# titoeb/RecModel

Hardware: AMD Instinct MI355X
Metric: ALS user+item row-updates/sec (higher is better)
Workload: dtype f32; 1 GPU; cfg3: WMF k=128+bias, 10000000x1000000 CSR, 99990947 nnz, alpha-log confidence, gamma=0.1, zipf_a=0.0; n_items=1000000, nnz=99990947, k=128, bias=True

## Files before the change

### include/wmf_hip.h

```cpp
#ifndef WMF_HIP_H
#define WMF_HIP_H

#include <stdint.h>

#ifdef __cplusplus
extern "C" {
#endif

#define WMF_OK            0
#define WMF_EINVAL       -1
#define WMF_EHIP         -2
#define WMF_ENOMEM       -3
#define WMF_ENUMERIC     -4

#define WMF_MAX_F        260

typedef struct wmf_plan wmf_plan;

const char* wmf_last_error(void);
int  wmf_version(void);
int  wmf_ld_for(int f);

int wmf_recompute_factors_host(const float* Y_host, int64_t m, int f, int bias,
                               const int64_t* indptr, const int32_t* indices, const float* values,
// ... 1 lines not shown

int64_t wmf_gram_workspace_bytes(int f);

int wmf_gram(const float* Y, int64_t m, int f, int ld, int bias,
             double* G_sum, void* workspace, void* stream);

int wmf_factorize(const double* G_sum, int f, int ld, double lambda,
                  float* W_white, float* W_unwhite, int32_t* info,
                  void* workspace, void* stream);

int wmf_rolled_layout_supported(int f, int ld);

int wmf_row_transform(const float* in, int64_t m, int f, int ld, const float* W,
                      int set_col0_one, float* out, float* col0_out, void* stream);
int wmf_whitened_row_floats(int f, int ld, int bias);

int  wmf_plan_create(const int64_t* indptr_host, int64_t n, int f, int bias, wmf_plan** out);
void wmf_plan_destroy(wmf_plan* p);
int  wmf_plan_stats(const wmf_plan* p, int64_t* out14);
int  wmf_plan_iter_stats(wmf_plan* p, int64_t* out4);

int wmf_solve_rows(const wmf_plan* plan, const float* V, const float* bias_fixed,
                   const int64_t* indptr, const int32_t* indices, const float* values,
                   int64_t n, int f, int ld, float* g, int32_t* fail_count, void* stream);
#define WMF_SOLVE_ROLLED 1
int wmf_solve_rows_ex(const wmf_plan* plan, const float* V, const float* bias_fixed,
                   const int64_t* indptr, const int32_t* indices, const float* values,
                   int64_t n, int f, int ld, float* g, int32_t* fail_count, int flags, void* stream);

int64_t wmf_eval_workspace_bytes(void);
// ... 133 lines not shown
```

### recmodel_amd/_lib.py

```python
import ctypes
import os

import torch

_HERE = os.path.dirname(os.path.abspath(__file__))
LIB_PATH = os.environ.get("WMF_HIP_LIB", os.path.join(_HERE, "libwmf_hip.so"))

WMF_OK, WMF_EINVAL, WMF_EHIP, WMF_ENOMEM, WMF_ENUMERIC = 0, -1, -2, -3, -4

c_int, c_i64, c_dbl, c_vp = ctypes.c_int, ctypes.c_int64, ctypes.c_double, ctypes.c_void_p

SIGNATURES = {
    "wmf_last_error": (ctypes.c_char_p, []),
    "wmf_version": (c_int, []),
    "wmf_ld_for": (c_int, [c_int]),
    "wmf_recompute_factors_host": (c_int, [c_vp, c_i64, c_int, c_int, c_vp, c_vp, c_vp, c_i64, c_dbl, c_vp]),
    "wmf_gram_workspace_bytes": (c_i64, [c_int]),
    "wmf_gram": (c_int, [c_vp, c_i64, c_int, c_int, c_int, c_vp, c_vp, c_vp]),
    "wmf_factorize": (c_int, [c_vp, c_int, c_int, c_dbl, c_vp, c_vp, c_vp, c_vp, c_vp]),
    "wmf_row_transform": (c_int, [c_vp, c_i64, c_int, c_int, c_vp, c_int, c_vp, c_vp, c_vp]),
    "wmf_whitened_row_floats": (c_int, [c_int, c_int, c_int]),
    "wmf_plan_create": (c_int, [c_vp, c_i64, c_int, c_int, ctypes.POINTER(c_vp)]),
    "wmf_plan_destroy": (None, [c_vp]),
    "wmf_plan_stats": (c_int, [c_vp, c_vp]),
    "wmf_plan_iter_stats": (c_int, [c_vp, c_vp]),
    "wmf_solve_rows": (c_int, [c_vp, c_vp, c_vp, c_vp, c_vp, c_vp, c_i64, c_int, c_int, c_vp, c_vp, c_vp]),
    "wmf_solve_rows_ex": (c_int, [c_vp, c_vp, c_vp, c_vp, c_vp, c_vp, c_i64, c_int, c_int, c_vp, c_vp, c_int, c_vp]),
    "wmf_rolled_layout_supported": (c_int, [c_int, c_int]),
    "wmf_eval_workspace_bytes": (c_i64, []),
    "wmf_eval_sqerr": (c_int, [c_vp, c_vp, c_int, c_int, c_int, c_vp, c_vp, c_vp, c_i64, c_vp, c_vp, c_vp]),
    "wmf_audit_workspace_bytes": (c_i64, [c_i64]),
    "wmf_half_step_audit": (c_int, [c_vp, c_vp, c_int, c_int, c_int, c_vp, c_vp, c_vp, c_i64, c_vp, c_vp, c_vp, c_vp, c_i64, c_vp]),
    "wmf_half_step_audit_f64": (c_int, [c_vp, c_vp, c_int, c_int, c_vp, c_vp, c_vp, c_i64, c_vp, c_vp, c_vp, c_vp, c_i64, c_vp]),
    "wmf_predict_pairs": (c_int, [c_vp, c_vp, c_int, c_int, c_int, c_vp, c_i64, c_vp, c_i64, c_vp, c_vp]),
    "wmf_partial_row_floats": (c_i64, [c_int]),
    "wmf_accumulate_rows": (c_int, [c_vp, c_vp, c_vp, c_vp, c_vp, c_vp, c_i64, c_i64, c_int, c_int, c_vp, c_int, c_int, c_vp, c_vp]),
# ... 130 lines not shown
```

### recmodel_amd/csrc/wmf_api.hip

```cpp
#include "../../include/wmf_hip.h"
#include "wmf_internal.h"

#include <atomic>
#include <cstdarg>
#include <cstdio>
#include <cstring>
#include <mutex>
#include <set>
#include <string>
#include <vector>

static thread_local char g_err[512] = "";
int wmf_debug_flags = 0;

void wmf_set_error(const char* fmt, ...) {
    va_list ap;
    va_start(ap, fmt);
    vsnprintf(g_err, sizeof(g_err), fmt, ap);
    va_end(ap);
}

#define HIP_TRY(call)                                                                            \
    do {                                                                                         \
        hipError_t e_ = (call);                                                                  \
// ... 197 lines not shown
    return check_launch("wmf_factorize");
}

int wmf_row_transform(const float* in, int64_t m, int f, int ld, const float* W, int set_col0_one, float* out,
                      float* col0_out, void* stream) {
    int rc = check_shape(f, ld);
    if (rc) return rc;
    if (!in || !W || !out || m < 0) { wmf_set_error("wmf_row_transform: null pointer or negative m"); return WMF_EINVAL; }
    rc = wmf_launch_transform(in, m, f, ld, W, set_col0_one, out, col0_out, (hipStream_t)stream);
    if (rc) {
        if (rc == WMF_L_LAYOUT) wmf_set_error("wmf_row_transform: f=%d, ld=%d with set_col0_one writes the split layout: col0_out (float[2 m]) is required and out may not alias in", f, ld);
        else wmf_set_error("wmf_row_transform: unsupported f=%d", f);
        return WMF_EINVAL;
    }
    return check_launch("wmf_row_transform");
}

static int bin_of(int64_t d, int f) {
    if (d <= 16) return WMF_BIN_LOW16;
    if (d <= 32) return WMF_BIN_LOW32;
    return wmf_direct_supported(f) ? WMF_BIN_MFMA : WMF_BIN_GENERAL;
}

int wmf_plan_create(const int64_t* indptr, int64_t n, int f, int bias, wmf_plan** out) {
    if (!indptr || !out || n < 0 || n > 0x7fffffffLL) { wmf_set_error("wmf_plan_create: bad arguments"); return WMF_EINVAL; }
    if (f < 1 || f > WMF_MAX_F) { wmf_set_error("wmf_plan_create: f=%d unsupported", f); return WMF_EINVAL; }
    wmf_plan* p = new wmf_plan();
    memset(p, 0, sizeof(*p));
    p->n = n; p->f = f;
    std::vector<int32_t> order((size_t)n);
// ... 558 lines not shown
```

### recmodel_amd/csrc/wmf_dense.hip

```cpp
#include "wmf_common.h"
#include "wmf_internal.h"

#include <type_traits>
#include <utility>

template <int NFB, int NSPLIT, int S>
__device__ __forceinline__ void gram_body(const float* __restrict__ Y, int64_t m, int f, int ld, int bias,
                                          float* __restrict__ partial, int64_t step_lo, int64_t step_hi) {
    constexpr int NT = NFB * (NFB + 1) / 2;
    constexpr int NACC = (NT + NSPLIT - 1) / NSPLIT;
    const int lane = threadIdx.x & 63;
    const int r = lane & 15, q = lane >> 4;
    f32x4 acc[NACC];
#pragma unroll
    for (int i = 0; i < NACC; ++i) acc[i] = f32x4{0.f, 0.f, 0.f, 0.f};

    constexpr int U = 4;
    float cur[U][NFB], nxt[U][NFB];
    const int last_col = min(16 * (NFB - 1) + r, ld - 1);
    const float col_mask_last = (16 * (NFB - 1) + r < f) ? 1.f : 0.f;
    auto load_trip = [&](int64_t s0, float (&fr)[U][NFB]) {
#pragma unroll
        for (int uu = 0; uu < U; ++uu) {
            const int64_t row = min(4 * (s0 + uu) + q, m - 1);
// ... 32 lines not shown
    float* out = partial + (int64_t)blockIdx.x * NT * 256;
    int t = 0;
#pragma unroll
    for (int bi = 0; bi < NFB; ++bi) {
#pragma unroll
        for (int bj = bi; bj < NFB; ++bj, ++t) {
            if (t % NSPLIT == S) {
#pragma unroll
                for (int reg = 0; reg < 4; ++reg) out[(t * 4 + reg) * 64 + lane] = acc[t / NSPLIT][reg];
            }
        }
    }
}

typedef __bf16 gram_bf16x8 __attribute__((ext_vector_type(8)));
template <int NFB>
__device__ __forceinline__ void gram_body6(const float* __restrict__ Y, int64_t m, int f, int ld, int bias,
                                           float* __restrict__ partial, int64_t step_lo, int64_t step_hi) {
    constexpr int NT = NFB * (NFB + 1) / 2;
    constexpr int NG1 = (5 * NFB + 4) / 9;
    const int lane = threadIdx.x;
    const int r = lane & 15, q = lane >> 4;
    f32x4 acc[NT];
#pragma unroll
    for (int i = 0; i < NT; ++i) acc[i] = f32x4{0.f, 0.f, 0.f, 0.f};
    const int last_col = min(16 * (NFB - 1) + r, ld - 1);
    const float col_mask_last = (16 * (NFB - 1) + r < f) ? 1.f : 0.f;
    const bool bias_lane = bias && r == 0;
    const int64_t stride = 32 * step_hi;
    auto load_blocks = [&](int64_t c0, float (&fr)[8][NFB], int fb_lo, int fb_hi) {
#pragma unroll
        for (int j = 0; j < 8; ++j) {
            const int64_t row = min(c0 + 8 * q + j, m - 1);
            const float* yrow = Y + row * (int64_t)ld;
#pragma unroll
            for (int fb = 0; fb < NFB; ++fb)
                if (fb >= fb_lo && fb < fb_hi) fr[j][fb] = yrow[fb == NFB - 1 ? last_col : 16 * fb + r];
        }
    };
    auto split = [&](int64_t c0, const float (&fr)[8][NFB], auto masked, gram_bf16x8 (&hi)[NFB], gram_bf16x8 (&mid)[NFB],
                     gram_bf16x8 (&lo)[NFB]) {
#pragma unroll
        for (int fb = 0; fb < NFB; ++fb) {
#pragma unroll
            for (int j = 0; j < 8; ++j) {
                const float rmask = (!decltype(masked)::value || c0 + 8 * q + j < m) ? 1.f : 0.f;
                float x = fr[j][fb];
                if (decltype(masked)::value) x *= rmask;
                if (fb == NFB - 1) x *= col_mask_last;
                if (fb == 0 && bias_lane) x = rmask;
                const __bf16 h = (__bf16)x;
                const float r1 = x - (float)h;
                const __bf16 md = (__bf16)r1;
                hi[fb][j] = h; mid[fb][j] = md; lo[fb][j] = (__bf16)(r1 - (float)md);
            }
        }
    };
    auto products = [&](const gram_bf16x8 (&hi)[NFB], const gram_bf16x8 (&mid)[NFB], const gram_bf16x8 (&lo)[NFB]) {
        int t0 = 0;
#pragma unroll
        for (int bi = 0; bi < NFB; ++bi) {
#pragma unroll
            for (int bj = bi; bj < NFB; ++bj) acc[t0 + bj - bi] = __builtin_amdgcn_mfma_f32_16x16x32_bf16(lo[bi], hi[bj], acc[t0 + bj - bi], 0, 0, 0);
#pragma unroll
            for (int bj = bi; bj < NFB; ++bj) acc[t0 + bj - bi] = __builtin_amdgcn_mfma_f32_16x16x32_bf16(mid[bi], mid[bj], acc[t0 + bj - bi], 0, 0, 0);
// ... 30 lines not shown
        gram_bf16x8 hi[NFB], mid[NFB], lo[NFB];
        split(c0, cur, std::true_type{}, hi, mid, lo);
        products(hi, mid, lo);
    }
    float* out = partial + (int64_t)blockIdx.x * NT * 256;
#pragma unroll
    for (int t = 0; t < NT; ++t)
#pragma unroll
        for (int reg = 0; reg < 4; ++reg) out[(t * 4 + reg) * 64 + lane] = acc[t][reg];
}

template <int NFB>
__global__ __launch_bounds__(64) void gram6_kernel(const float* __restrict__ Y, int64_t m, int f, int ld, int bias,
                                                   float* __restrict__ partial, int64_t steps_per_wave) {
    gram_body6<NFB>(Y, m, f, ld, bias, partial, blockIdx.x, gridDim.x);
}

template <int NFB, int NSPLIT>
__global__ __launch_bounds__(NSPLIT == 1 ? 64 : 256) void gram_kernel(const float* __restrict__ Y, int64_t m, int f, int ld, int bias,
                                                  float* __restrict__ partial, int64_t steps_per_wave) {
    const int64_t nsteps = (m + 3) / 4;
    int64_t lo = (int64_t)blockIdx.x * steps_per_wave;
    int64_t hi = lo + steps_per_wave;
    if (hi > nsteps) hi = nsteps;
    if (lo > hi) lo = hi;
    if constexpr (NSPLIT == 1) {
        gram_body<NFB, 1, 0>(Y, m, f, ld, bias, partial, lo, hi);
    } else {
        switch (__builtin_amdgcn_readfirstlane(threadIdx.x >> 6)) {
            case 0: gram_body<NFB, NSPLIT, 0>(Y, m, f, ld, bias, partial, lo, hi); break;
// ... 68 lines not shown
    const int cap = wmf_gram_max_waves(f);
    if (want > cap) want = cap;
    if (want > 1024) want -= want % 1024;
    return (int)want;
}

int wmf_launch_gram(const float* Y, int64_t m, int f, int ld, int bias, double* G_sum, float* partial, double* slices,
                    hipStream_t st) {
    if (m <= 0) return hipMemsetAsync(G_sum, 0, (size_t)f * f * sizeof(double), st) == hipSuccess ? WMF_L_OK : WMF_L_NO_KERNEL;
    const int nfb = (f + 15) / 16;
    const int nwaves = wmf_gram_nwaves(m, f);
    if (const int rc = wmf_dispatch_nfb<1, 17>(nfb, [&](auto n) { return launch_gram_nfb<decltype(n)::value>(Y, m, f, ld, bias, partial, nwaves, st); })) return rc;
    WMF_LAUNCH("gram_reduce1_kernel", gram_reduce1_kernel, dim3((f * f + 255) / 256, WMF_GRAM_SLICES), dim3(256), 0, st, partial,
               nwaves, f, nfb, slices);
    WMF_LAUNCH("gram_reduce2_kernel", gram_reduce2_kernel, dim3((f * f + 255) / 256), dim3(256), 0, st, slices, f, G_sum);
    return WMF_L_OK;
}

__device__ __forceinline__ double rl_f64(double v, int lane) {
    const int lo = __builtin_amdgcn_readlane(__double2loint(v), lane);
    const int hi = __builtin_amdgcn_readlane(__double2hiint(v), lane);
    return __hiloint2double(hi, lo);
}

typedef double f64x4 __attribute__((ext_vector_type(4)));
#define WMF_MFMA16_F64(a, b, c) __builtin_amdgcn_mfma_f64_16x16x4f64((a), (b), (c), 0, 0, 0)
constexpr int FZ_LD = 66;

__device__ __forceinline__ f64x4 fz_mul_abt(const double* A, int la, const double* B, int lb, f64x4 c, int r, int q, double sign) {
#pragma unroll
// ... 516 lines not shown
    return WMF_L_OK;
}

int wmf_launch_transform(const float* in, int64_t m, int f, int ld, const float* W, int set_col0_one, float* out,
                         float* col0_out, hipStream_t st) {
    if (m <= 0) return WMF_L_OK;
    const int nfb = (f + 15) / 16;
    if (set_col0_one == 3 || set_col0_one == 4) {
        if (!wmf_rolled_layout(f, ld)) return WMF_L_NO_KERNEL;
    } else {
        set_col0_one = set_col0_one ? (wmf_split_layout(f, ld) ? 2 : 1) : 0;
    }
    if ((set_col0_one == 2 || set_col0_one == 3) && (!col0_out || in == out)) return WMF_L_LAYOUT;
    return wmf_dispatch_nfb<1, 17>(nfb, [&](auto n) { return launch_transform_nfb<decltype(n)::value>(in, m, f, ld, W, set_col0_one, out, col0_out, st); });
}
```

### recmodel_amd/csrc/wmf_internal.h

```cpp
#pragma once
#include <hip/hip_runtime.h>
#include <stdint.h>
#include <type_traits>
#include <utility>
#include "../../include/wmf_hip.h"

#define WMF_GRAM_MAX_WAVES 4096
#define WMF_EVAL_MAX_BLOCKS 2048
#define WMF_AUDIT_MAX_BLOCKS 2048
#define WMF_HEAVY_T 4096
#define WMF_SEG 2048
#define WMF_WIDE_LU_GRID 64

extern int wmf_debug_flags;
#ifdef WMF_LAB
constexpr bool WMF_LAB_BUILD = true;
#else
constexpr bool WMF_LAB_BUILD = false;
#endif
constexpr int WMF_DBG_SHIPPED = WMF_DBG_HEAVY_REG_RING | WMF_DBG_F32_GRAM | WMF_DBG_HEAVY_ONE_WAVE | WMF_DBG_F64_NO_LOW_RANK |
                                WMF_DBG_NO_ITER | WMF_DBG_F64_VALU;
constexpr int WMF_DBG_LAB = WMF_DBG_NO_ELIMINATION | WMF_DBG_NO_ACCUMULATION | WMF_DBG_NO_TILE_INVERSE | WMF_DBG_LOW32_GAUSS_JORDAN |
                            WMF_DBG_NO_BORDER | WMF_DBG_WIDE_EIGHT_WAVES | WMF_DBG_NO_ROW_PAIRS | WMF_DBG_HEAVY_F32_ACC |
                            WMF_DBG_HEAVY_REG_RING_K64 | WMF_DBG_F32_TRANSFORM | WMF_DBG_LOW_F32_TILES | WMF_DBG_WIDE_F32 |
// ... 24 lines not shown
    int64_t iter_count, iter_nnz;
    int iter_dmax;
    int32_t* iter_bounce_rows;
    int32_t* iter_info;
    unsigned long long* iter_stats;
};

int wmf_gram_max_waves(int f);
int wmf_gram_nwaves(int64_t m, int f);
int wmf_launch_gram(const float* Y, int64_t m, int f, int ld, int bias, double* G_sum, float* partial, double* slices,
                    hipStream_t st);
int wmf_launch_factorize(const double* G_sum, int f, int ld, double lambda, float* Wwhite, float* Wunwhite,
                         int32_t* info, double* gA, hipStream_t st);
int wmf_launch_transform(const float* in, int64_t m, int f, int ld, const float* W, int set_col0_one, float* out,
                         float* col0_out, hipStream_t st);

enum WmfLaunchRc { WMF_L_OK = 0, WMF_L_NO_KERNEL = -1, WMF_L_HIP = -2, WMF_L_LAYOUT = -3, WMF_L_TOO_MANY_KEYS = -4 };

struct RowArgs {
    const float* V; const float* side; const float* biasv; int bstride;
    const int64_t* indptr; const int32_t* indices; const float* vals;
    int f, ld; float* g; int32_t* fb_rows; int32_t* fb_count; int32_t* fail_count;
    int dbg; bool rolled; hipStream_t st;
};
struct RowList { const int32_t* rows; int64_t count; const int32_t* count_dev; };

template <int N>
using wmf_int = std::integral_constant<int, N>;
template <int... NS, class Fn>
static inline int wmf_dispatch_list(int n, Fn&& fn) {
// ... 152 lines not shown
```

### recmodel_amd/engine.py

```python
import ctypes
import os

import numpy as np
import torch

from . import _lib


def _ptr(t):
    return ctypes.c_void_p(t.data_ptr()) if t is not None else None


def _stream():
    return ctypes.c_void_p(torch.cuda.current_stream().cuda_stream)


class _HeldWork:

    def __init__(self, work, *buffers, landing=None):
        self.work, self.buffers, self.landing = work, buffers, landing

    def wait(self):
        self.work.wait()
        if self.landing is not None:
# ... 18 lines not shown
        return int(self.lib.wmf_gram_workspace_bytes(f))

    def eval_workspace_bytes(self):
        return int(self.lib.wmf_eval_workspace_bytes())

    def gram(self, Y, m, f, ld, bias, G, ws):
        _lib.check(self.lib.wmf_gram(_ptr(Y), m, f, ld, int(bias), _ptr(G), _ptr(ws), _stream()))

    def factorize(self, G, f, ld, lam, W_white, W_unwhite, info, ws):
        _lib.check(self.lib.wmf_factorize(_ptr(G), f, ld, float(lam), _ptr(W_white), _ptr(W_unwhite), _ptr(info), _ptr(ws),
                                          _stream()))

    def row_transform(self, inp, m, f, ld, W, set_col0_one, out, col0_out):
        _lib.check(self.lib.wmf_row_transform(_ptr(inp), m, f, ld, _ptr(W), int(set_col0_one), _ptr(out), _ptr(col0_out),
                                              _stream()))

    def plan_create(self, indptr_host, n, f, bias):
        handle = ctypes.c_void_p()
        _lib.check(self.lib.wmf_plan_create(indptr_host.ctypes.data_as(ctypes.c_void_p), n, f, int(bool(bias)), ctypes.byref(handle)))
        stats = np.zeros(14, dtype=np.int64)
        _lib.check(self.lib.wmf_plan_stats(handle, stats.ctypes.data_as(ctypes.c_void_p)))
        return handle, stats

    def plan_iter_stats(self, handle):
        out = np.zeros(4, dtype=np.int64)
        _lib.check(self.lib.wmf_plan_iter_stats(handle, out.ctypes.data_as(ctypes.c_void_p)))
        return out

    def plan_destroy(self, handle):
        self.lib.wmf_plan_destroy(handle)
# ... 234 lines not shown


def row_cost(degrees, f):
    return degrees.to(torch.float64) * float(f * f) + float(f) ** 3


def gathered_positions(ids, world, rows_per_rank, chunk_len, owner=None, local=None):
    j = ids // world if local is None else local
    r = ids % world if owner is None else owner
    s_c = (j // chunk_len) * chunk_len
    rest = rows_per_rank - s_c
    len_c = torch.clamp(rest, max=chunk_len) if torch.is_tensor(rest) else min(chunk_len, rest)
    return world * s_c + r * len_c + (j - s_c)


class AlsEngine:

    def __init__(self, n_users, n_items, dim, bias, gamma, device=None, group=None, kernels=None, chunks=None,
                 reduce_mode=None, pipe_mode=None, force_exchange=None, sparse_mode=None):
        self.K = kernels if kernels is not None else HipKernels()
        self.lib = getattr(self.K, "lib", None)
        self.device = torch.device(device if device is not None else f"cuda:{torch.cuda.current_device()}")
        self.group = group
        if group is not None or (torch.distributed.is_available() and torch.distributed.is_initialized()):
            self.world = torch.distributed.get_world_size(group)
            self.rank = torch.distributed.get_rank(group)
        else:
            self.world, self.rank = 1, 0
        if force_exchange is None:
            force_exchange = os.environ.get("WMF_FORCE_EXCHANGE") == "1"
        self.exchange = self.world > 1 or (bool(force_exchange) and torch.distributed.is_available()
                                           and torch.distributed.is_initialized())
        self.n = {"users": int(n_users), "items": int(n_items)}
        self.dim, self.bias, self.gamma = int(dim), bool(bias), float(gamma)
        self.f = self.dim + 1 if self.bias else self.dim
        self.ld = self.K.ld_for(self.f)
        self.pr = self.K.partial_row_floats(self.f) if hasattr(self.K, "partial_row_floats") else 0
        self._reduce_arg, self.pipe_mode, self._chunks_arg, self._sparse_arg = reduce_mode, pipe_mode, chunks, sparse_mode
        self.csr = {}
        self.csr_chunks = {}
        self._configure({s: Sharding(self.n[s], self.world, self.rank) for s in self.n})

    def _configure(self, shard):
        W = self.world
        self.shard = shard
        self.rpr = {s: shard[s].rpr for s in self.n}
        self.n_local = {s: shard[s].n_local for s in self.n}
        pr, chunks = self.pr, self._chunks_arg
        forced = os.environ.get("WMF_REDUCE") if self._reduce_arg is None else ("1" if self._reduce_arg else "0")
        self.reduce = {}
        for s in self.n:
            o = "items" if s == "users" else "users"
# ... 8 lines not shown
        want = {s: max(1, int(chunks)) for s in self.n}
        if auto_chunks:
            want = {s: max(1, min(want[s], (self.rpr[s] * (W if self.reduce[s] else 1)) // MIN_CHUNK_ROWS)) for s in self.n}
            for s in self.n:
                if self.reduce["items" if s == "users" else "users"]:
                    want[s] = 1
        self.chunk_len = {s: max(1, (self.rpr[s] + want[s] - 1) // want[s]) for s in self.n}
        self.chunk_bounds = {s: [(lo, min(self.chunk_len[s], self.rpr[s] - lo))
                                 for lo in range(0, max(self.rpr[s], 1), self.chunk_len[s]) if lo < self.rpr[s]]
                             for s in self.n}
        self.chunk_range = {s: [(W * lo, W * (lo + ln)) for lo, ln in self.chunk_bounds[s]] for s in self.n}
        self.sparse = {s: False for s in self.n}
        self.need = {}
        dev, f32 = self.device, torch.float32
        z = lambda *shape, dtype=f32: torch.zeros(*shape, dtype=dtype, device=dev)
        self.factors = {s: z(self.rpr[s], self.ld) for s in self.n}
        self.g = {s: z(self.rpr[s], self.ld) for s in self.n}
        self.X = {s: (z(W * self.rpr[s], self.ld) if self.exchange else self.factors[s]) for s in self.n}
        self._pending = {s: [] for s in self.n}
        self.ldv = self.K.whitened_row_floats(self.f, self.ld, self.bias)
        self.split = self.ldv != self.ld
        self.rolled = bool(self.split and self.bias and os.environ.get("WMF_ROLLED", "1") != "0"
                           and self.K.rolled_layout_supported(self.f, self.ld))
        self.white_mode = 3 if self.rolled else self.bias
        self.unwhite_mode = 4 if self.rolled else False
        self.solve_flags = 1 if self.rolled else 0
        self.V = {s: z(W * self.rpr[s], self.ldv) for s in self.n}
        self.bias_vec = {s: (z(W * self.rpr[s], 2) if self.split else z(W * self.rpr[s])) for s in self.n}
        self.G = z(self.f * self.f, dtype=torch.float64)
        self.W_white, self.W_unwhite = z(self.f, self.ld), z(self.f, self.ld)
        self.info = z(4, dtype=torch.int32)
        self.fail = z(4, dtype=torch.int32)
        self.ws = torch.empty(self.K.gram_workspace_bytes(self.f), dtype=torch.uint8, device=dev)
        self.eval_ws = torch.empty(self.K.eval_workspace_bytes(), dtype=torch.uint8, device=dev)
        self.eval_out = z(3, dtype=torch.float64)
        self.pipe = {s: False for s in self.n}
        self.csr_pipe = {}
        self.partial_pipe = {}
        self.csr_red = {}
        self.partial_all = {s: (torch.empty(W * self.rpr[s], pr, dtype=f32, device=dev) if self.reduce[s] else None) for s in self.n}
        self.partial_mine = {s: (torch.empty(self.rpr[s], pr, dtype=f32, device=dev) if self.reduce[s] else None) for s in self.n}
        self.scratch_rows = torch.zeros(max(self.rpr.values()), dtype=torch.int32, device=dev)
        self._stale = {s: False for s in self.n}
        self.csr, self.csr_chunks = {}, {}
        self.has_factors = {"users": False, "items": False}

    def positions(self, side, ids):
        sh = self.shard[side]
# ... 220 lines not shown
        indptr, idx, v = coo_to_csr(o.indices.to(torch.int64), local_rows, o.values, self.world * self.rpr[side], self.K, o.n_rows)
        deg = (indptr[1:] - indptr[:-1]).to(torch.int32).contiguous()
        w_eff = torch.empty_like(v) if self.bias and not self.split else None
        return indptr.contiguous(), deg, idx.contiguous(), v.contiguous(), w_eff

    def _shard(self, side, rows, cols, vals, plan=True):
        other = self._other(side)
        local = self.shard[side].local_of(rows)
        indptr, idx, v = coo_to_csr(local, self.positions(other, cols), vals, self.rpr[side], self.K, self.world * self.rpr[other])
        return Csr(self.K, indptr, idx, v, self.world * self.rpr[other], self.f, self.bias, plan=plan)

    def set_factors(self, side, full):
        full = torch.as_tensor(full, dtype=torch.float32)
        sh = self.shard[side]
        mine = (full[self.rank::self.world] if sh.owner is None else full[sh.my_ids(full.device)]).to(self.device)
        blk = self.factors[side]
        blk.zero_()
        blk[: mine.shape[0], : self.f] = mine
        self.has_factors[side] = True
        for c in range(len(self.chunk_bounds[side])):
            self._publish(side, c)

    def get_factors(self, side):
        ids = torch.arange(self.n[side], device=self.device)
        if self.sparse[side]:
            W = self.world
            self._wait(side)
            dense = torch.zeros(W * self.rpr[side], self.ld, dtype=torch.float32, device=self.device)
            for lo, ln in self.chunk_bounds[side]:
                torch.distributed.all_gather_into_tensor(dense[W * lo: W * (lo + ln)], self.factors[side][lo: lo + ln].contiguous(),
# ... 31 lines not shown
        return _HeldWork(work, send_h, landing=(out, out_h))

    def _ensure_gathered(self, side):
        if self._stale[side]:
            self._stale[side] = False
            for c in range(len(self.chunk_bounds[side])):
                self._publish(side, c, force=True)
        self._wait(side)

    def _wait(self, side):
        for work in self._pending[side]:
            if work is not None:
                work.wait()
        self._pending[side] = []

    def prepare(self, fixed):
        K = self.K
        blk = self.factors[fixed]
        K.gram(blk, self.n_local[fixed], self.f, self.ld, self.bias, self.G, self.ws)
        if self.exchange:
            torch.distributed.all_reduce(self.G, group=self.group)
        K.factorize(self.G, self.f, self.ld, self.gamma, self.W_white, self.W_unwhite, self.info, self.ws)
        V, bvec = self.V[fixed], self.bias_vec[fixed]
        if not self.exchange:
            K.row_transform(self.X[fixed], self.n_local[fixed], self.f, self.ld, self.W_white, self.white_mode, V,
                            bvec if self.bias else None)
            return
        if self._stale[fixed]:
            self._ensure_gathered(fixed)
        pending, self._pending[fixed] = self._pending[fixed], []
        done = len(self.chunk_bounds[fixed]) - len(pending)
        for c, (start, stop) in enumerate(self.chunk_range[fixed]):
            if c >= done and pending[c - done] is not None:
                pending[c - done].wait()
            rows = slice(start, stop)
            if stop > start:
                K.row_transform(self.X[fixed][rows], stop - start, self.f, self.ld, self.W_white, self.white_mode, V[rows],
                                bvec[rows] if self.bias else None)

    def update(self, side):
        K = self.K
        fixed = self._other(side)
        bvec = self.bias_vec[fixed] if self.bias else None
        self._wait(side)
        for c, ((lo, ln), csr) in enumerate(zip(self.chunk_bounds[side], self.csr_chunks[side])):
            g = self.g[side][lo: lo + ln]
            K.solve_rows(csr._plan, self.V[fixed], bvec, csr.indptr, csr.indices, csr.values, ln, self.f, self.ld, g, self.fail,
                         self.solve_flags)
            real = max(0, min(ln, self.n_local[side] - lo))
            K.row_transform(g, real, self.f, self.ld, self.W_unwhite, self.unwhite_mode, self.factors[side][lo: lo + ln], None)
            self._publish(side, c)
        self.has_factors[side] = True

    def half_step(self, side):
        if self.reduce[side]:
            return self._half_step_reduce(side)
        if self.pipe[side]:
            return self._half_step_pipelined(side)
        self.prepare(self._other(side))
        self.update(side)

    def _half_step_pipelined(self, side):
        K, W = self.K, self.world
        fixed = self._other(side)
        K.gram(self.factors[fixed], self.n_local[fixed], self.f, self.ld, self.bias, self.G, self.ws)
        torch.distributed.all_reduce(self.G, group=self.group)
# ... 81 lines not shown
        self.update(side)

    def _reduce_scatter(self, out, inp):
        if torch.distributed.get_backend(self.group) == "nccl":
            return torch.distributed.reduce_scatter_tensor(out, inp, group=self.group, async_op=True)
        torch.distributed.all_reduce(inp, group=self.group)
        n = out.shape[0]
        out.copy_(inp[self.rank * n: (self.rank + 1) * n])
        return None

    def half_step_unweighted(self, side):
        K = self.K
        fixed = self._other(side)
        self.prepare(fixed)
        c = self.csr[side]
        K.spmm_rows(self.V[fixed], c.indptr, c.indices, c.values, c.n_rows, self.f, self.ld, self.g[side])
        K.row_transform(self.g[side], self.n_local[side], self.f, self.ld, self.W_unwhite, self.unwhite_mode, self.factors[side], None)
        self.has_factors[side] = True
        for c in range(len(self.chunk_bounds[side])):
            self._publish(side, c)

    @property
    def iter_on(self):
        return not (_lib.load().wmf_debug_get_flags() & _lib.DEBUG_FLAGS["WMF_DBG_NO_ITER"])

    def iter_stats(self, side):
        out = np.zeros(4, dtype=np.int64)
        for c in self.csr_chunks.get(side, []):
            out += c.iter_stats()
        return out
# ... 77 lines not shown
```

Measured before the change: 422.1 million row-updates/s.

## Chain whitening transforms from solver outputs and defer factor materialization

Instead of unwhitening each solved row into factors and then re-reading those factors for the next half-step's Gram and whitening transform, the engine keeps the whitened solutions g plus the unwhitening matrix U. It computes an augmented Gram of g, composes U into the next whitening matrix on a small dense path, and applies one combined transform from g directly to V. The per-row unwhitening pass over the solved side is skipped and only materialized lazily when factors are accessed. This removes a full read/write pass over the factor matrix per half-step, at the cost of extra small compose kernels, a lazy-materialization wrapper, and possible numerical drift from the chained transforms.

After: 454.4 million row-updates/s, median of 6. 7.6% higher.

```diff
diff --git a/include/wmf_hip.h b/include/wmf_hip.h
--- a/include/wmf_hip.h
+++ b/include/wmf_hip.h
@@ -39,6 +39,15 @@
 int wmf_row_transform(const float* in, int64_t m, int f, int ld, const float* W,
                       int set_col0_one, float* out, float* col0_out, void* stream);
 int wmf_whitened_row_floats(int f, int ld, int bias);
+
+int wmf_chained_supported(int f, int ld, int bias);
+int wmf_gram_whitened(const float* g, int64_t m, int f, int ld, int bias,
+                      double* G_aug, void* workspace, void* stream);
+int wmf_compose_whitening(const double* G_aug, const float* U, int f, int ld, int bias, int rolled, double lambda,
+                          float* W_white, float* W_unwhite, float* N_ext, int32_t* info,
+                          void* workspace, void* stream);
+int wmf_row_transform_chained(const float* g, int64_t m, int f, int ld, int bias, const float* N_ext, int rolled,
+                              float* out, float* col0_out, void* stream);
 
 int  wmf_plan_create(const int64_t* indptr_host, int64_t n, int f, int bias, wmf_plan** out);
 void wmf_plan_destroy(wmf_plan* p);
diff --git a/recmodel_amd/_lib.py b/recmodel_amd/_lib.py
--- a/recmodel_amd/_lib.py
+++ b/recmodel_amd/_lib.py
@@ -20,6 +20,10 @@
     "wmf_factorize": (c_int, [c_vp, c_int, c_int, c_dbl, c_vp, c_vp, c_vp, c_vp, c_vp]),
     "wmf_row_transform": (c_int, [c_vp, c_i64, c_int, c_int, c_vp, c_int, c_vp, c_vp, c_vp]),
     "wmf_whitened_row_floats": (c_int, [c_int, c_int, c_int]),
+    "wmf_chained_supported": (c_int, [c_int, c_int, c_int]),
+    "wmf_gram_whitened": (c_int, [c_vp, c_i64, c_int, c_int, c_int, c_vp, c_vp, c_vp]),
+    "wmf_compose_whitening": (c_int, [c_vp, c_vp, c_int, c_int, c_int, c_int, c_dbl, c_vp, c_vp, c_vp, c_vp, c_vp, c_vp]),
+    "wmf_row_transform_chained": (c_int, [c_vp, c_i64, c_int, c_int, c_int, c_vp, c_int, c_vp, c_vp, c_vp]),
     "wmf_plan_create": (c_int, [c_vp, c_i64, c_int, c_int, ctypes.POINTER(c_vp)]),
     "wmf_plan_destroy": (None, [c_vp]),
     "wmf_plan_stats": (c_int, [c_vp, c_vp]),
diff --git a/recmodel_amd/csrc/wmf_api.hip b/recmodel_amd/csrc/wmf_api.hip
--- a/recmodel_amd/csrc/wmf_api.hip
+++ b/recmodel_amd/csrc/wmf_api.hip
@@ -235,6 +235,60 @@
         return WMF_EINVAL;
     }
     return check_launch("wmf_row_transform");
+}
+
+int wmf_chained_supported(int f, int ld, int bias) {
+    if (check_shape(f, ld)) return 0;
+    const int f1 = f + (bias ? 1 : 0);
+    return (f >= 97 && f1 <= 144 && ld >= f1 && f + 1 <= WMF_MAX_F) ? 1 : 0;
+}
+static int check_chained(const char* what, int f, int ld, int bias) {
+    if (wmf_chained_supported(f, ld, bias)) return WMF_OK;
+    wmf_set_error("%s: unsupported f=%d, ld=%d, bias=%d (wmf_chained_supported)", what, f, ld, bias);
+    return WMF_EINVAL;
+}
+
+int wmf_gram_whitened(const float* g, int64_t m, int f, int ld, int bias, double* G_aug, void* workspace, void* stream) {
+    if (check_chained("wmf_gram_whitened", f, ld, bias)) return WMF_EINVAL;
+    if (!g || !G_aug || !workspace || m < 0) { wmf_set_error("wmf_gram_whitened: null pointer or negative m"); return WMF_EINVAL; }
+    {
+        const int f1 = f + (bias ? 1 : 0);
+        const int64_t nfb = (f1 + 15) / 16, nt = nfb * (nfb + 1) / 2;
+        if ((int64_t)wmf_gram_nwaves(m, f1) * nt * 256 * (int64_t)sizeof(float) > gram_partial_bytes(f + 1)) {
+            wmf_set_error("wmf_gram_whitened: workspace layout too small at f=%d", f);
+            return WMF_EINVAL;
+        }
+    }
+    if (wmf_launch_gram_aug(g, m, f, ld, bias, G_aug, (float*)workspace, (double*)((char*)workspace + gram_slices_off(f + 1)),
+                            (hipStream_t)stream)) {
+        wmf_set_error("wmf_gram_whitened: unsupported f=%d", f);
+        return WMF_EINVAL;
+    }
+    return check_launch("wmf_gram_whitened");
+}
+
+int wmf_compose_whitening(const double* G_aug, const float* U, int f, int ld, int bias, int rolled, double lambda, float* W_white,
+                          float* W_unwhite, float* N_ext, int32_t* info, void* workspace, void* stream) {
+    if (check_chained("wmf_compose_whitening", f, ld, bias)) return WMF_EINVAL;
+    if (!G_aug || !U || !W_white || !W_unwhite || !N_ext || !info || !workspace) { wmf_set_error("wmf_compose_whitening: null pointer"); return WMF_EINVAL; }
+    if (rolled && !(bias && wmf_rolled_layout(f, ld))) { wmf_set_error("wmf_compose_whitening: rolled needs wmf_rolled_layout_supported(f=%d, ld=%d) and bias", f, ld); return WMF_EINVAL; }
+    if (U == W_unwhite || U == W_white) { wmf_set_error("wmf_compose_whitening: U may not alias an output"); return WMF_EINVAL; }
+    wmf_launch_compose(G_aug, U, f, ld, bias, rolled, lambda, W_white, W_unwhite, N_ext, info, (double*)workspace,
+                       (double*)((char*)workspace + gram_a_off(f + 1)), (hipStream_t)stream);
+    return check_launch("wmf_compose_whitening");
+}
+
+int wmf_row_transform_chained(const float* g, int64_t m, int f, int ld, int bias, const float* N_ext, int rolled, float* out,
+                              float* col0_out, void* stream) {
+    if (check_chained("wmf_row_transform_chained", f, ld, bias)) return WMF_EINVAL;
+    if (!g || !N_ext || !out || m < 0) { wmf_set_error("wmf_row_transform_chained: null pointer or negative m"); return WMF_EINVAL; }
+    const int rc = wmf_launch_transform_chained(g, m, f, ld, bias, N_ext, rolled, out, col0_out, (hipStream_t)stream);
+    if (rc) {
+        if (rc == WMF_L_LAYOUT) wmf_set_error("wmf_row_transform_chained: f=%d, ld=%d: col0_out is required with biases and out may not alias g in the split layout", f, ld);
+        else wmf_set_error("wmf_row_transform_chained: unsupported f=%d, ld=%d, rolled=%d", f, ld, rolled);
+        return WMF_EINVAL;
+    }
+    return check_launch("wmf_row_transform_chained");
 }
 
 static int bin_of(int64_t d, int f) {
diff --git a/recmodel_amd/csrc/wmf_dense.hip b/recmodel_amd/csrc/wmf_dense.hip
--- a/recmodel_amd/csrc/wmf_dense.hip
+++ b/recmodel_amd/csrc/wmf_dense.hip
@@ -70,7 +70,7 @@
 }
 
 typedef __bf16 gram_bf16x8 __attribute__((ext_vector_type(8)));
-template <int NFB>
+template <int NFB, bool AUG = false>
 __device__ __forceinline__ void gram_body6(const float* __restrict__ Y, int64_t m, int f, int ld, int bias,
                                            float* __restrict__ partial, int64_t step_lo, int64_t step_hi) {
     constexpr int NT = NFB * (NFB + 1) / 2;
@@ -82,7 +82,8 @@
     for (int i = 0; i < NT; ++i) acc[i] = f32x4{0.f, 0.f, 0.f, 0.f};
     const int last_col = min(16 * (NFB - 1) + r, ld - 1);
     const float col_mask_last = (16 * (NFB - 1) + r < f) ? 1.f : 0.f;
-    const bool bias_lane = bias && r == 0;
+    const bool bias_lane = bias && r == (AUG ? (f - 1) & 15 : 0);
+    constexpr int ONE_FB = AUG ? NFB - 1 : 0;
     const int64_t stride = 32 * step_hi;
     auto load_blocks = [&](int64_t c0, float (&fr)[8][NFB], int fb_lo, int fb_hi) {
 #pragma unroll
@@ -103,8 +104,8 @@
                 const float rmask = (!decltype(masked)::value || c0 + 8 * q + j < m) ? 1.f : 0.f;
                 float x = fr[j][fb];
                 if (decltype(masked)::value) x *= rmask;
-                if (fb == NFB - 1) x *= col_mask_last;
-                if (fb == 0 && bias_lane) x = rmask;
+                if (fb == NFB - 1) x = AUG ? (col_mask_last != 0.f ? x : 0.f) : x * col_mask_last;
+                if (fb == ONE_FB && bias_lane) x = rmask;
                 const __bf16 h = (__bf16)x;
                 const float r1 = x - (float)h;
                 const __bf16 md = (__bf16)r1;
@@ -165,6 +166,12 @@
 __global__ __launch_bounds__(64) void gram6_kernel(const float* __restrict__ Y, int64_t m, int f, int ld, int bias,
                                                    float* __restrict__ partial, int64_t steps_per_wave) {
     gram_body6<NFB>(Y, m, f, ld, bias, partial, blockIdx.x, gridDim.x);
+}
+
+template <int NFB>
+__global__ __launch_bounds__(64) void gram6_aug_kernel(const float* __restrict__ g, int64_t m, int f1, int ld, int bias,
+                                                       float* __restrict__ partial) {
+    gram_body6<NFB, true>(g, m, f1, ld, bias, partial, blockIdx.x, gridDim.x);
 }
 
 template <int NFB, int NSPLIT>
@@ -263,6 +270,24 @@
     WMF_LAUNCH("gram_reduce1_kernel", gram_reduce1_kernel, dim3((f * f + 255) / 256, WMF_GRAM_SLICES), dim3(256), 0, st, partial,
                nwaves, f, nfb, slices);
     WMF_LAUNCH("gram_reduce2_kernel", gram_reduce2_kernel, dim3((f * f + 255) / 256), dim3(256), 0, st, slices, f, G_sum);
+    return WMF_L_OK;
+}
+
+int wmf_launch_gram_aug(const float* g, int64_t m, int f, int ld, int bias, double* G_aug, float* partial, double* slices,
+                        hipStream_t st) {
+    const int f1 = f + (bias ? 1 : 0), nfb = (f1 + 15) / 16;
+    if (nfb < 7 || nfb > 9) return WMF_L_NO_KERNEL;
+    if (m <= 0) return hipMemsetAsync(G_aug, 0, (size_t)f1 * f1 * sizeof(double), st) == hipSuccess ? WMF_L_OK : WMF_L_NO_KERNEL;
+    const int nwaves = wmf_gram_nwaves(m, f1);
+    if (const int rc = wmf_dispatch_nfb<7, 9>(nfb, [&](auto n) {
+            constexpr int NFB = decltype(n)::value;
+            static const char* nm = wmf_kname("gram6_aug_kernel<%d>", NFB);
+            WMF_LAUNCH(nm, (gram6_aug_kernel<NFB>), dim3(nwaves), dim3(64), 0, st, g, m, f1, ld, bias, partial);
+            return (int)WMF_L_OK;
+        })) return rc;
+    WMF_LAUNCH("gram_reduce1_kernel", gram_reduce1_kernel, dim3((f1 * f1 + 255) / 256, WMF_GRAM_SLICES), dim3(256), 0, st, partial,
+               nwaves, f1, nfb, slices);
+    WMF_LAUNCH("gram_reduce2_kernel", gram_reduce2_kernel, dim3((f1 * f1 + 255) / 256), dim3(256), 0, st, slices, f1, G_aug);
     return WMF_L_OK;
 }
 
@@ -809,3 +834,236 @@
     if ((set_col0_one == 2 || set_col0_one == 3) && (!col0_out || in == out)) return WMF_L_LAYOUT;
     return wmf_dispatch_nfb<1, 17>(nfb, [&](auto n) { return launch_transform_nfb<decltype(n)::value>(in, m, f, ld, W, set_col0_one, out, col0_out, st); });
 }
+
+__device__ __forceinline__ double compose_t(const float* __restrict__ U, int f, int ld, int bias, int rolled, int p, int j) {
+    if (p >= f) return j == 0 ? 1.0 : 0.0;
+    if (bias && j == 0) return 0.0;
+    const int src = rolled ? (p + 1 == f ? 0 : p + 1) : p;
+    return (double)U[src * ld + j];
+}
+template <class FA, class FB>
+__device__ __forceinline__ double compose_dot16(int n, FA a, FB b) {
+    double s = 0.0;
+#pragma unroll 3
+    for (int k = threadIdx.x & 15; k < n; k += 16) s += a(k) * b(k);
+#pragma unroll
+    for (int off = 8; off; off >>= 1) s += __shfl_xor(s, off, 16);
+    return s;
+}
+__global__ __launch_bounds__(256) void compose_h_kernel(const double* __restrict__ Gaug, const float* __restrict__ U, int f, int ld,
+                                                        int bias, int rolled, double* __restrict__ H) {
+    const int f1 = f + (bias ? 1 : 0);
+    const int e0 = (blockIdx.x * blockDim.x + threadIdx.x) >> 4;
+    const bool live = e0 < f1 * f;
+    const int e = live ? e0 : 0;
+    const int p = e / f, j = e - p * f;
+    const double s = compose_dot16(f1, [&](int k) { return Gaug[p * f1 + k]; }, [&](int k) { return compose_t(U, f, ld, bias, rolled, k, j); });
+    if (live && (threadIdx.x & 15) == 0) H[e] = s;
+}
+__global__ __launch_bounds__(256) void compose_g_kernel(const double* __restrict__ H, const float* __restrict__ U, int f, int ld,
+                                                        int bias, int rolled, double* __restrict__ Gt) {
+    const int f1 = f + (bias ? 1 : 0);
+    const int e0 = (blockIdx.x * blockDim.x + threadIdx.x) >> 4;
+    const bool live = e0 < f * f;
+    const int e = live ? e0 : 0;
+    int i = e / f, j = e - i * f;
+    if (i > j) { const int t = i; i = j; j = t; }
+    const double s = compose_dot16(f1, [&](int p) { return compose_t(U, f, ld, bias, rolled, p, i); }, [&](int p) { return H[p * f + j]; });
+    if (live && (threadIdx.x & 15) == 0) Gt[e] = s;
+}
+__global__ __launch_bounds__(256) void compose_n_kernel(const float* __restrict__ U, const float* __restrict__ Ww, int f, int ld,
+                                                        int bias, int rolled, float* __restrict__ N) {
+    const int f1 = f + (bias ? 1 : 0);
+    const int e0 = (blockIdx.x * blockDim.x + threadIdx.x) >> 4;
+    const bool live = e0 < f1 * ld;
+    const int e = live ? e0 : 0;
+    const int p = e / ld, n = e - p * ld;
+    const int col = n >= f ? 0 : rolled ? (n + 1 == f ? 0 : n + 1) : n;
+    double s = compose_dot16(f, [&](int j) { return compose_t(U, f, ld, bias, rolled, p, j); }, [&](int j) { return (double)Ww[j * ld + col]; });
+    if (n >= f) s = (n == f && bias && p < f) ? (double)U[(rolled ? (p + 1 == f ? 0 : p + 1) : p) * ld] : 0.0;
+    if (live && (threadIdx.x & 15) == 0) N[e] = (float)s;
+}
+
+int wmf_launch_compose(const double* G_aug, const float* U, int f, int ld, int bias, int rolled, double lambda, float* Wwhite,
+                       float* Wunwhite, float* N_ext, int32_t* info, double* scratch, double* gA, hipStream_t st) {
+    const int f1 = f + (bias ? 1 : 0);
+    double* H = scratch;
+    double* Gt = scratch + (size_t)f1 * f;
+    WMF_LAUNCH("compose_h_kernel", compose_h_kernel, dim3((f1 * f + 15) / 16), dim3(256), 0, st, G_aug, U, f, ld, bias, rolled, H);
+    WMF_LAUNCH("compose_g_kernel", compose_g_kernel, dim3((f * f + 15) / 16), dim3(256), 0, st, H, U, f, ld, bias, rolled, Gt);
+    wmf_launch_factorize(Gt, f, ld, lambda, Wwhite, Wunwhite, info, gA, st);
+    WMF_LAUNCH("compose_n_kernel", compose_n_kernel, dim3((f1 * ld + 15) / 16), dim3(256), 0, st, U, Wwhite, f, ld, bias, rolled, N_ext);
+    return WMF_L_OK;
+}
+
+template <int NFB, int MODE>
+__global__ __launch_bounds__(512) void chain6_kernel(const float* __restrict__ in, int64_t m, int f, int ld,
+                                                     const float* __restrict__ W,
+                                                     float* __restrict__ out, float* __restrict__ col0_out,
+                                                     int64_t nblocks16) {
+    extern __shared__ __attribute__((aligned(16))) char smem_raw[];
+    constexpr int NP = 16 * NFB;
+    constexpr int NKC = (NP + 31) / 32;
+    constexpr int KS = 176;
+    static_assert(32 * NKC <= KS, "K does not fit the LDS row");
+    __bf16* Wt = reinterpret_cast<__bf16*>(smem_raw);
+    __shared__ int nz[NKC * NFB];
+    const int tid = threadIdx.x;
+    constexpr bool bias = MODE != 0;
+    const int f1 = f + (bias ? 1 : 0);
+    for (int e = tid; e < NKC * NFB; e += 512) nz[e] = 0;
+    __syncthreads();
+    typedef __bf16 stage_bf16x8 __attribute__((ext_vector_type(8)));
+    stage_bf16x8* Ws = reinterpret_cast<stage_bf16x8*>(Wt);
+    for (int it = tid; it < NP * (KS / 8); it += 512) {
+        const int k8 = it / NP, n = it - k8 * NP;
+        float v[8];
+#pragma unroll
+        for (int j = 0; j < 8; ++j) {
+            const int k = 8 * k8 + j;
+            const bool in_w = k < f1 && n < f1;
+            v[j] = W[in_w ? k * ld + n : 0];
+            if (!in_w) v[j] = 0.f;
+        }
+        stage_bf16x8 ph, pm, pl;
+        bool any = false;
+#pragma unroll
+        for (int j = 0; j < 8; ++j) {
+            const __bf16 h = (__bf16)v[j];
+            const float r1 = v[j] - (float)h;
+            const __bf16 md = (__bf16)r1;
+            ph[j] = h; pm[j] = md; pl[j] = (__bf16)(r1 - (float)md);
+            any |= v[j] != 0.f;
+        }
+        const int at = (n * KS + 8 * k8) / 8;
+        Ws[at] = ph;
+        Ws[NP * KS / 8 + at] = pm;
+        Ws[2 * NP * KS / 8 + at] = pl;
+        if (any) nz[(k8 >> 2) * NFB + (n >> 4)] = 1;
+    }
+    __syncthreads();
+    const int lane = tid & 63, wv = __builtin_amdgcn_readfirstlane(tid >> 6);
+    const int r = lane & 15, q = lane >> 4;
+    const int nch = ld >> 2;
+    unsigned cmask[NKC];
+#pragma unroll
+    for (int c = 0; c < NKC; ++c) {
+        unsigned mk = 0;
+#pragma unroll
+        for (int nb = 0; nb < NFB; ++nb) mk |= nz[c * NFB + nb] ? (1u << nb) : 0u;
+        cmask[c] = __builtin_amdgcn_readfirstlane(mk);
+    }
+    typedef __bf16 bf16x8_t __attribute__((ext_vector_type(8)));
+    const bf16x8_t* Wl = reinterpret_cast<const bf16x8_t*>(Wt);
+    const int64_t stride = (int64_t)gridDim.x * 8;
+    auto request = [&](int64_t blk, float4 (&x)[2 * NKC]) {
+        const int64_t row = blk * 16 + r;
+        const float4* irow = reinterpret_cast<const float4*>(in + (row < m ? row : 0) * (int64_t)ld);
+#pragma unroll
+        for (int c = 0; c < NKC; ++c) {
+            x[2 * c] = irow[min(8 * c + 2 * q, nch - 1)];
+            x[2 * c + 1] = irow[min(8 * c + 2 * q + 1, nch - 1)];
+        }
+    };
+    constexpr bool sp = MODE == 2 || MODE == 3;
+    const int fcol = f & 15;
+    auto block = [&](int64_t blk, float4 (&xc)[2 * NKC]) {
+        f32x4 acc[NFB];
+#pragma unroll
+        for (int nb = 0; nb < NFB; ++nb) acc[nb] = f32x4{0.f, 0.f, 0.f, 0.f};
+#pragma unroll
+        for (int c = 0; c < NKC; ++c) {
+            const int k0 = 32 * c + 8 * q;
+            float xe[8] = {xc[2 * c].x, xc[2 * c].y, xc[2 * c].z, xc[2 * c].w, xc[2 * c + 1].x, xc[2 * c + 1].y, xc[2 * c + 1].z, xc[2 * c + 1].w};
+            if (32 * c + 32 > 16 * (NFB - 1)) {
+#pragma unroll
+                for (int e = 0; e < 8; ++e) if (!(k0 + e < f)) xe[e] = (bias && k0 + e == f) ? 1.f : 0.f;
+            }
+            bf16x8_t ah, am, al;
+#pragma unroll
+            for (int e = 0; e < 8; ++e) {
+                const __bf16 h = (__bf16)xe[e];
+                const float r1 = xe[e] - (float)h;
+                const __bf16 md = (__bf16)r1;
+                ah[e] = h; am[e] = md; al[e] = (__bf16)(r1 - (float)md);
+            }
+            unsigned mv = cmask[c];
+            asm volatile("" : "+v"(mv));
+            const unsigned mk = __builtin_amdgcn_readfirstlane(mv);
+#pragma unroll
+            for (int nb = 0; nb < NFB; ++nb) {
+                if (!(mk & (1u << nb))) continue;
+                const int at = ((16 * nb + r) * KS + 32 * c + 8 * q) / 8;
+                const bf16x8_t bh = Wl[at], bm = Wl[NP * KS / 8 + at], bl = Wl[2 * NP * KS / 8 + at];
+                f32x4 cc = acc[nb];
+                cc = __builtin_amdgcn_mfma_f32_16x16x32_bf16(al, bh, cc, 0, 0, 0);
+                cc = __builtin_amdgcn_mfma_f32_16x16x32_bf16(am, bm, cc, 0, 0, 0);
+                cc = __builtin_amdgcn_mfma_f32_16x16x32_bf16(ah, bl, cc, 0, 0, 0);
+                cc = __builtin_amdgcn_mfma_f32_16x16x32_bf16(am, bh, cc, 0, 0, 0);
+                cc = __builtin_amdgcn_mfma_f32_16x16x32_bf16(ah, bm, cc, 0, 0, 0);
+                cc = __builtin_amdgcn_mfma_f32_16x16x32_bf16(ah, bh, cc, 0, 0, 0);
+                acc[nb] = cc;
+            }
+        }
+        const int wid = sp ? f - 1 : ld;
+        const bool stuff = MODE == 3 && (r & 7) < 2;
+        const int stuff_sh = 2 * (r >> 3) + (r & 7);
+        auto store_rows = [&](auto full) {
+#pragma unroll
+            for (int reg = 0; reg < 4; ++reg) {
+                const int64_t orow = blk * 16 + 4 * q + reg;
+                const float bias_src = acc[NFB - 1][reg];
+                const unsigned bbits = MODE == 3 ? (unsigned)__builtin_amdgcn_ds_bpermute((16 * q + fcol) * 4, __builtin_bit_cast(int, bias_src)) : 0u;
+                if (decltype(full)::value || orow < m) {
+                    float* o = out + orow * (int64_t)wid;
+#pragma unroll
+                    for (int nb = 0; nb < NFB; ++nb) {
+                        const int col = 16 * nb + r;
+                        float v = acc[nb][reg];
+                        if (MODE == 3 && 16 * nb < 128) {
+                            const unsigned vb = __builtin_bit_cast(unsigned, v);
+                            v = __builtin_bit_cast(float, stuff ? ((vb & ~1u) | ((bbits >> (4 * nb + stuff_sh)) & 1u)) : vb);
+                        }
+                        if (nb < NFB - 1) { o[col] = v; continue; }
+                        if (col < wid) o[col] = col < f ? v : 0.f;
+                        else if (sp && col == f - 1) col0_out[2 * orow] = v;
+                        if (bias && col == f) col0_out[sp ? 2 * orow + 1 : orow] = v;
+                    }
+                }
+            }
+        };
+        if (blk * 16 + 16 <= m) store_rows(std::true_type{});
+        else store_rows(std::false_type{});
+    };
+    float4 xa[2 * NKC];
+    for (int64_t blk = (int64_t)blockIdx.x * 8 + wv; blk < nblocks16; blk += stride) {
+        request(blk, xa);
+        block(blk, xa);
+    }
+}
+
+int wmf_launch_transform_chained(const float* g, int64_t m, int f, int ld, int bias, const float* N_ext, int rolled, float* out,
+                                 float* col0_out, hipStream_t st) {
+    if (m <= 0) return WMF_L_OK;
+    const int f1 = f + (bias ? 1 : 0), nfb = (f1 + 15) / 16;
+    if (nfb < 7 || nfb > 9) return WMF_L_NO_KERNEL;
+    if (rolled && !(bias && wmf_rolled_layout(f, ld))) return WMF_L_NO_KERNEL;
+    const int mode = !bias ? 0 : rolled ? 3 : wmf_split_layout(f, ld) ? 2 : 1;
+    if (bias && !col0_out) return WMF_L_LAYOUT;
+    if (g == out && mode >= 2) return WMF_L_LAYOUT;
+    const int64_t nblk = (m + 15) / 16;
+    int64_t grid = (nblk + 7) / 8;
+    if (grid > wmf_cu_count()) grid = wmf_cu_count();
+    if (grid < 1) grid = 1;
+    return wmf_dispatch_nfb<7, 9>(nfb, [&](auto n) {
+        constexpr int NFB = decltype(n)::value;
+        return wmf_dispatch_nfb<0, 3>(mode, [&](auto md) {
+            constexpr int MODE = decltype(md)::value;
+            constexpr size_t lds = (size_t)3 * 16 * NFB * 176 * 2;
+            static const char* nm = wmf_kname("chain6_kernel<%d, %d>", NFB, MODE);
+            WMF_LAUNCH_LDS(nm, (chain6_kernel<NFB, MODE>), lds, dim3((unsigned)grid), dim3(512), lds, st, g, m, f, ld, N_ext, out,
+                           col0_out, nblk);
+            return (int)WMF_L_OK;
+        });
+    });
+}
diff --git a/recmodel_amd/csrc/wmf_internal.h b/recmodel_amd/csrc/wmf_internal.h
--- a/recmodel_amd/csrc/wmf_internal.h
+++ b/recmodel_amd/csrc/wmf_internal.h
@@ -62,6 +62,12 @@
                          int32_t* info, double* gA, hipStream_t st);
 int wmf_launch_transform(const float* in, int64_t m, int f, int ld, const float* W, int set_col0_one, float* out,
                          float* col0_out, hipStream_t st);
+int wmf_launch_gram_aug(const float* g, int64_t m, int f, int ld, int bias, double* G_aug, float* partial, double* slices,
+                        hipStream_t st);
+int wmf_launch_compose(const double* G_aug, const float* U, int f, int ld, int bias, int rolled, double lambda, float* Wwhite,
+                       float* Wunwhite, float* N_ext, int32_t* info, double* scratch, double* gA, hipStream_t st);
+int wmf_launch_transform_chained(const float* g, int64_t m, int f, int ld, int bias, const float* N_ext, int rolled, float* out,
+                                 float* col0_out, hipStream_t st);
 
 enum WmfLaunchRc { WMF_L_OK = 0, WMF_L_NO_KERNEL = -1, WMF_L_HIP = -2, WMF_L_LAYOUT = -3, WMF_L_TOO_MANY_KEYS = -4 };
 
diff --git a/recmodel_amd/engine.py b/recmodel_amd/engine.py
--- a/recmodel_amd/engine.py
+++ b/recmodel_amd/engine.py
@@ -56,6 +56,20 @@
     def row_transform(self, inp, m, f, ld, W, set_col0_one, out, col0_out):
         _lib.check(self.lib.wmf_row_transform(_ptr(inp), m, f, ld, _ptr(W), int(set_col0_one), _ptr(out), _ptr(col0_out),
                                               _stream()))
+
+    def chained_supported(self, f, ld, bias):
+        return bool(self.lib.wmf_chained_supported(f, ld, int(bias)))
+
+    def gram_whitened(self, g, m, f, ld, bias, G_aug, ws):
+        _lib.check(self.lib.wmf_gram_whitened(_ptr(g), m, f, ld, int(bias), _ptr(G_aug), _ptr(ws), _stream()))
+
+    def compose_whitening(self, G_aug, U, f, ld, bias, rolled, lam, W_white, W_unwhite, N_ext, info, ws):
+        _lib.check(self.lib.wmf_compose_whitening(_ptr(G_aug), _ptr(U), f, ld, int(bias), int(rolled), float(lam), _ptr(W_white),
+                                                  _ptr(W_unwhite), _ptr(N_ext), _ptr(info), _ptr(ws), _stream()))
+
+    def row_transform_chained(self, g, m, f, ld, bias, N_ext, rolled, out, col0_out):
+        _lib.check(self.lib.wmf_row_transform_chained(_ptr(g), m, f, ld, int(bias), _ptr(N_ext), int(rolled), _ptr(out),
+                                                      _ptr(col0_out), _stream()))
 
     def plan_create(self, indptr_host, n, f, bias):
         handle = ctypes.c_void_p()
@@ -320,10 +334,33 @@
     return world * s_c + r * len_c + (j - s_c)
 
 
+class _SideBuffers(dict):
+
+    def __init__(self, engine, data):
+        super().__init__(data)
+        self._engine = engine
+
+    def raw(self, side):
+        return dict.__getitem__(self, side)
+
+    def __getitem__(self, side):
+        self._engine._materialize(side)
+        return dict.__getitem__(self, side)
+
+    def get(self, side, default=None):
+        return self[side] if side in self else default
+
+    def values(self):
+        return [self[s] for s in self]
+
+    def items(self):
+        return [(s, self[s]) for s in self]
+
+
 class AlsEngine:
 
     def __init__(self, n_users, n_items, dim, bias, gamma, device=None, group=None, kernels=None, chunks=None,
-                 reduce_mode=None, pipe_mode=None, force_exchange=None, sparse_mode=None):
+                 reduce_mode=None, pipe_mode=None, force_exchange=None, sparse_mode=None, chained=True):
         self.K = kernels if kernels is not None else HipKernels()
         self.lib = getattr(self.K, "lib", None)
         self.device = torch.device(device if device is not None else f"cuda:{torch.cuda.current_device()}")
@@ -342,6 +379,9 @@
         self.f = self.dim + 1 if self.bias else self.dim
         self.ld = self.K.ld_for(self.f)
         self.pr = self.K.partial_row_floats(self.f) if hasattr(self.K, "partial_row_floats") else 0
+        self._fixed_from_g = False
+        self.chained = bool(chained and not self.exchange and hasattr(self.K, "row_transform_chained")
+                            and self.K.chained_supported(self.f, self.ld, self.bias))
         self._reduce_arg, self.pipe_mode, self._chunks_arg, self._sparse_arg = reduce_mode, pipe_mode, chunks, sparse_mode
         self.csr = {}
         self.csr_chunks = {}
@@ -380,9 +420,11 @@
         self.need = {}
         dev, f32 = self.device, torch.float32
         z = lambda *shape, dtype=f32: torch.zeros(*shape, dtype=dtype, device=dev)
-        self.factors = {s: z(self.rpr[s], self.ld) for s in self.n}
+        self._owed = {s: False for s in self.n}
+        self.g_valid = {s: False for s in self.n}
+        self.factors = _SideBuffers(self, {s: z(self.rpr[s], self.ld) for s in self.n})
         self.g = {s: z(self.rpr[s], self.ld) for s in self.n}
-        self.X = {s: (z(W * self.rpr[s], self.ld) if self.exchange else self.factors[s]) for s in self.n}
+        self.X = _SideBuffers(self, {s: (z(W * self.rpr[s], self.ld) if self.exchange else self.factors.raw(s)) for s in self.n})
         self._pending = {s: [] for s in self.n}
         self.ldv = self.K.whitened_row_floats(self.f, self.ld, self.bias)
         self.split = self.ldv != self.ld
@@ -397,7 +439,12 @@
         self.W_white, self.W_unwhite = z(self.f, self.ld), z(self.f, self.ld)
         self.info = z(4, dtype=torch.int32)
         self.fail = z(4, dtype=torch.int32)
-        self.ws = torch.empty(self.K.gram_workspace_bytes(self.f), dtype=torch.uint8, device=dev)
+        self.ws = torch.empty(self.K.gram_workspace_bytes(self.f + 1 if self.chained else self.f), dtype=torch.uint8, device=dev)
+        if self.chained:
+            f1 = self.f + (1 if self.bias else 0)
+            self.U = {s: z(self.f, self.ld) for s in self.n}
+            self.G_aug = z(f1 * f1, dtype=torch.float64)
+            self.N_ext = z(f1, self.ld)
         self.eval_ws = torch.empty(self.K.eval_workspace_bytes(), dtype=torch.uint8, device=dev)
         self.eval_out = z(3, dtype=torch.float64)
         self.pipe = {s: False for s in self.n}
@@ -648,6 +695,7 @@
         full = torch.as_tensor(full, dtype=torch.float32)
         sh = self.shard[side]
         mine = (full[self.rank::self.world] if sh.owner is None else full[sh.my_ids(full.device)]).to(self.device)
+        self._invalidate(side)
         blk = self.factors[side]
         blk.zero_()
         blk[: mine.shape[0], : self.f] = mine
@@ -709,8 +757,28 @@
                 work.wait()
         self._pending[side] = []
 
+    def _invalidate(self, side):
+        self.g_valid[side] = self._owed[side] = False
+
+    def _materialize(self, side):
+        if self._owed[side]:
+            self._owed[side] = False
+            self.K.row_transform(self.g[side], self.n_local[side], self.f, self.ld, self.U[side], self.unwhite_mode,
+                                 self.factors.raw(side), None)
+
+    def _prepare_chained(self, fixed):
+        K, n = self.K, self.n_local[fixed]
+        K.gram_whitened(self.g[fixed], n, self.f, self.ld, self.bias, self.G_aug, self.ws)
+        K.compose_whitening(self.G_aug, self.U[fixed], self.f, self.ld, self.bias, self.rolled, self.gamma, self.W_white,
+                            self.W_unwhite, self.N_ext, self.info, self.ws)
+        K.row_transform_chained(self.g[fixed], n, self.f, self.ld, self.bias, self.N_ext, self.rolled, self.V[fixed],
+                                self.bias_vec[fixed] if self.bias else None)
+
     def prepare(self, fixed):
         K = self.K
+        self._fixed_from_g = self.chained and self.g_valid[fixed]
+        if self._fixed_from_g:
+            return self._prepare_chained(fixed)
         blk = self.factors[fixed]
         K.gram(blk, self.n_local[fixed], self.f, self.ld, self.bias, self.G, self.ws)
         if self.exchange:
@@ -738,13 +806,20 @@
         fixed = self._other(side)
         bvec = self.bias_vec[fixed] if self.bias else None
         self._wait(side)
+        self._invalidate(side)
         for c, ((lo, ln), csr) in enumerate(zip(self.chunk_bounds[side], self.csr_chunks[side])):
             g = self.g[side][lo: lo + ln]
             K.solve_rows(csr._plan, self.V[fixed], bvec, csr.indptr, csr.indices, csr.values, ln, self.f, self.ld, g, self.fail,
                          self.solve_flags)
+            if self.chained and self._fixed_from_g:
+                continue
             real = max(0, min(ln, self.n_local[side] - lo))
-            K.row_transform(g, real, self.f, self.ld, self.W_unwhite, self.unwhite_mode, self.factors[side][lo: lo + ln], None)
+            K.row_transform(g, real, self.f, self.ld, self.W_unwhite, self.unwhite_mode, self.factors.raw(side)[lo: lo + ln], None)
             self._publish(side, c)
+        if self.chained:
+            self.U[side].copy_(self.W_unwhite)
+            self.g_valid[side] = True
+            self._owed[side] = self._fixed_from_g
         self.has_factors[side] = True
 
     def half_step(self, side):
@@ -856,6 +931,7 @@
         fixed = self._other(side)
         self.prepare(fixed)
         c = self.csr[side]
+        self._invalidate(side)
         K.spmm_rows(self.V[fixed], c.indptr, c.indices, c.values, c.n_rows, self.f, self.ld, self.g[side])
         K.row_transform(self.g[side], self.n_local[side], self.f, self.ld, self.W_unwhite, self.unwhite_mode, self.factors[side], None)
         self.has_factors[side] = True
```
